# dguilliams3/book-recommendation-engine

Hardware: AMD Instinct MI355X
Metric: exact top-10 queries/sec at 10M×1536 fp32 (1/8 GPU) + % HBM/MFMA roofline (higher is better)
Workload: dtype fp32

## Files before the change

### book-recommendation-engine_amd/csrc/vs_engines.hip

```cpp
#include "vs_host.h"

using namespace vs;
using namespace vs::host;

namespace {

bool env_on(const char* name) {
  const char* e = getenv(name);
  return !e || atoi(e) != 0;
}
int env_int(const char* name, int dflt) {
  const char* e = getenv(name);
  return e ? atoi(e) : dflt;
}

int engine_from_env() {
  const char* e = getenv("VS_ENGINE");
  if (!e) return VS_ENGINE_AUTO;
  if (strcmp(e, "fp32") == 0) return VS_ENGINE_FP32_MFMA;
  if (strcmp(e, "bf16v") == 0) return VS_ENGINE_BF16_VERIFY;
  if (strcmp(e, "i8v") == 0) return VS_ENGINE_I8_VERIFY;
  return VS_ENGINE_AUTO;
}
bool wide_enabled() {
// ... 318 lines not shown
    if (!gathered) x.timing = &tm;
    if (gathered && s.deep && !i8 && s.kmode == MODE_IP && a.self0 < 0 && skinny_deep_on()) {
      VS_HIP(launch_skinny_plane(FILTER_BF16, x.XH, x.QH, x.ld, s.ntotal, s.gc, nullptr, nullptr,
                                 s.part, st),
             "vs: skinny deep stage");
      x.qskip = skinny_plane_max_queries();
    }
    if (s.small) {
      int* cnt = nullptr;
      VS_HIP(s.scr.alloc((void**)&cnt, sizeof(int)), "vs: scratch");
      VS_HIP(hipMemsetD32Async((hipDeviceptr_t)cnt, a.nq, 1, st), "vs: count");
      KernelTimer ks(st, i8 ? "skinny_plane_topk_i8" : "skinny_plane_topk");
      VS_HIP(launch_skinny_plane(s.plane, x.XH, x.QH, x.ld, s.ntotal, cnt, s.qs, x.xs, s.part, st,
                                 a.nq),
             "vs: skinny first stage");
      ks.stop();
    } else {
      int nd = 0;
      VS_HIP(launch_gemm_topk_x1(s.kmode, x, s.part, st, &nd), "vs: gemm_topk_x1 launch");
    }
    x.timing = nullptr;
    whole.stop();
  }
  if (s.aug)
    VS_HIP(launch_l2aug_map(s.part.key, s.part.id, (int64_t)s.part.P * s.part.KP, s.qa_rows,
                            s.qaux, s.idx->aug.nref, x.qcut, st),
           "vs: L2 keys");
  return VS_OK;
}

int merge_and_verify(Stage& s) {
  vs_index* idx = s.idx;
  const SearchArgs& a = s.a;
  Scratch& scr = s.scr;
  hipStream_t st = s.st;
  const Partials& part = s.part;
  const int nq = s.nq, KF = s.KF, L = s.L;
  float* Dk = nullptr;
  int64_t* Ik = nullptr;
  VS_HIP(scr.alloc((void**)&Dk, (size_t)nq * KF * sizeof(float)), "vs: scratch");
  VS_HIP(scr.alloc((void**)&Ik, (size_t)nq * KF * sizeof(int64_t)), "vs: scratch");
  if (KF > 64) {
    VS_HIP(launch_select_lists(part, L, nq, KF, Dk, Ik, st, s.gc), "vs: merge");
  } else if (select_heads_applies(part, L, KF)) {
    VS_HIP(launch_select_heads(part, nq, KF, Dk, Ik, st, s.gc), "vs: merge");
  } else {
    Partials mp = part;
    mp.KP = kp_for(KF);
    mp.KL = L;
    VS_HIP(launch_merge_partials(MODE_L2, mp, nq, KF, 0, 0.0f, Dk, Ik, KF, st, 0, nullptr, s.gc),
           "vs: merge");
  }
  Partials vp;
  vp.KP = kp_for(KF);
  vp.P = 1;
  int* flags = nullptr;
  VS_HIP(scr.alloc((void**)&vp.key, (size_t)nq * vp.KP * sizeof(float)), "vs: scratch");
  VS_HIP(scr.alloc((void**)&vp.id, (size_t)nq * vp.KP * sizeof(int)), "vs: scratch");
  VS_HIP(scr.alloc((void**)&flags, (size_t)nq * sizeof(int)), "vs: scratch");
  VS_HIP(scr.alloc((void**)&s.qlist, (size_t)s.x.nq_pad * sizeof(int)), "vs: scratch");
  VS_HIP(scr.alloc((void**)&s.qcount, 2 * sizeof(int)), "vs: scratch");
  VerifyArgs v;
  v.mode = s.vmode;
  v.KF = KF;
  v.M = s.need;
  v.X = idx->codes;
  v.xesize = idx->esize;
  v.xn = idx->norms;
  v.Q = s.Q;
  v.qn = s.qaux;
  v.ld = idx->ld;
  v.ba = s.ba;
  v.stats = s.stats;
  v.lists = part;
  v.L = L;
  v.okey = vp.key;
  v.oid = vp.id;
  v.KP = vp.KP;
  v.fail = flags;
  v.qinv = a.mode == MODE_COS ? s.qaux : nullptr;
  v.xinv = a.mode == MODE_COS ? a.xaux : nullptr;
  v.qr2i8 = s.qr2;
  v.qcut = s.x.qcut;
  VS_HIP(launch_verify_rescore(v, nq, Dk, Ik, s.gc, st), "vs: verify");
  unsigned long long* dst = device_stats(idx->device);
  if (!dst) return fail(VS_E_HIP, "vs: statistics buffer");
  VS_HIP(launch_compact_flags(flags, nq, s.qlist, s.qcount, dst + 1,
                              s.gathered ? nullptr : dst + 0, st),
         "vs: flags");
  if (wide_enabled())
    VS_HIP(launch_verify_wide(v, nq, s.qlist, s.qcount, Dk, Ik, dst + 4, st), "vs: verify wide");
  VS_HIP(launch_compact_flags(flags, nq, s.qlist, s.qcount + 1,
                              s.last_plane ? dst + 2 : dst + 3, nullptr, st),
         "vs: flags");
  VS_HIP(launch_merge_partials(s.vmode, vp, nq, a.k, idx->id_base, a.min_score, a.D, a.I, a.k, st,
                               a.raw, s.gl, s.gc),
         "vs: merge");
  return VS_OK;
}

int hand_off(Stage& s) {
  vs_index* idx = s.idx;
  const SearchArgs& a = s.a;
  hipStream_t st = s.st;
  const int* left_count = s.qcount + 1;
  int left = -1;
  if ((!s.gathered || s.deep) && tail_wait_on(a, st)) {
    int rc = read_count(left_count, st, &left);
    if (rc) return rc;
  }
  if (!s.last_plane && !s.gathered && s.plane == FILTER_I8) {
    int rc = adaptive_record(idx, left_count, s.nq, st);
    if (rc) return rc;
  }
  if (left == 0) return VS_OK;
  const int* next = s.qlist;
  if (s.gathered) {
    int* composed = nullptr;
    VS_HIP(s.scr.alloc((void**)&composed, (size_t)s.x.nq_pad * sizeof(int)), "vs: scratch");
    VS_HIP(launch_compose_list(s.gl, s.qlist, left_count, s.x.nq_pad, composed, st), "vs: flags");
    next = composed;
  }
  if (!s.last_plane)
    return run_filter_verify(idx, a, s.need, s.KF, st, FILTER_BF16, true, true, next, left_count);
  return run_gemm_rescored(idx, a, s.need, s.KF, s.plane, st, next, left_count);
}

int run_filter_verify(vs_index* idx, const SearchArgs& a, int need, int KF, hipStream_t st,
                      int plane, bool last_plane, bool deep, const int* gl, const int* gc) {
  Stage s(idx, a, need, KF, st, plane, last_plane, deep, gl, gc);
  int rc = size_lists(s);
  if (!rc) rc = stage_queries(s);
  if (!rc) rc = arm_dumps(s);
  if (!rc) rc = run_pass(s);
  if (!rc) rc = merge_and_verify(s);
  if (!rc) rc = hand_off(s);
  return rc;
}

constexpr int kExactSlots = 256;
constexpr int kXPageSlots = 1024;

int run_gemm_rescored(vs_index* idx, const SearchArgs& a, int need, int KF, int plane,
                      hipStream_t st, const int* gl, const int* gc) {
  if (KF > 64) return run_paged(idx, a, st, gl, gc);
  const int ntotal = (int)idx->ntotal;
  const int KP = kp_for(KF);
  const int nslot = (int)round_up(a.nq, kBQ);
  Partials part;
  part.KP = KP;
  const int ntiles = (ntotal + kBN - 1) / kBN;
  const int nsplit = gathered_nsplit(ntiles);
  part.P = 2 * nsplit;
  const int cap = slot_window_cap(nslot, part.P, KP);
  Scratch scr(st);
  const size_t n = (size_t)cap * part.P * KP;
  VS_HIP(scr.alloc((void**)&part.key, n * sizeof(float)), "vs: scratch");
  VS_HIP(scr.alloc((void**)&part.id, n * sizeof(int)), "vs: scratch");
  float *qc = nullptr, *ac = nullptr;
  int* qrow = nullptr;
  VS_HIP(scr.alloc((void**)&qc, (size_t)cap * idx->ld * sizeof(float)), "vs: scratch");
  VS_HIP(scr.alloc((void**)&ac, (size_t)cap * sizeof(float)), "vs: scratch");
  VS_HIP(scr.alloc((void**)&qrow, (size_t)cap * sizeof(int)), "vs: scratch");
  float* Dk = nullptr;
  int64_t* Ik = nullptr;
  VS_HIP(scr.alloc((void**)&Dk, (size_t)cap * KF * sizeof(float)), "vs: scratch");
// ... 424 lines not shown
```

### book-recommendation-engine_amd/csrc/vs_internal.h

```cpp
#pragma once

#include <hip/hip_runtime.h>

#include <cfloat>
#include <climits>
#include <cstdint>

namespace vs {

enum Mode : int { MODE_IP = 0, MODE_L2 = 1, MODE_COS = 2, MODE_L2D = 3 };

constexpr int kBN = 128;
constexpr int kBQ = 128;
constexpr int kBK = 32;
constexpr int kRowPad = 256;
constexpr int kGemvMaxQ = 8;
constexpr int kBlasThreshold = 20;
constexpr int kSkinnyMaxQ = 32;

__host__ __device__ inline uint16_t f32_to_bf16_rne(float f) {
  uint32_t u;
  __builtin_memcpy(&u, &f, 4);
  if ((u & 0x7F800000u) == 0x7F800000u && (u & 0x007FFFFFu))
    return (uint16_t)((u >> 16) | 0x0040u);
// ... 36 lines not shown
  virtual void end(hipStream_t st) = 0;
  virtual ~X1Timing() = default;
};
struct X1Args {
  X1Timing* timing = nullptr;
  int qskip = 0;
  int filter = FILTER_BF16;
  const void* XH = nullptr;
  const float* xs = nullptr;
  const float* xgmax = nullptr;
  const float* xgmin = nullptr;
  bool dump = false;
  bool dump32 = false;
  float* qcut = nullptr;
  const double* qbkey = nullptr;
  int qcut_m = 0;
  int recut = 1;
  const float* ecut_x = nullptr;
  const float* ecut_q = nullptr;
  int64_t ecut_ld = 0;
  float* qam = nullptr;
  float* ecut_key = nullptr;
  int* ecut_id = nullptr;
  int* dcount = nullptr;
  int* dslot = nullptr;
  int dR = 0;
  unsigned long long* dstats = nullptr;
  const float* xaux = nullptr;
  const void* QH = nullptr;
  int qtile0 = 0;
  const float* qs = nullptr;
  const float* qaux = nullptr;
  int nqa = 0;
  int64_t ld = 0;
  int ntotal = 0;
  int nq_pad = 0;
  int nsplit = 1;
  int64_t self0 = -1;
  const int* qrow = nullptr;
  const int* qcount = nullptr;
};
constexpr int kX1Q = 256;
constexpr int kEcutMaxM = 32;
constexpr int64_t kI8MaxLd = 131072;
int x1_list_len(int need);
int x1_lane_len();
hipError_t x1_stamps(unsigned long long* out, int reset);
bool x1_plan_describe(int mode, int filter, int64_t ntotal, int nsplit, bool can_dump, bool ecut,
                      bool gathered, int recut, bool dump32, int32_t* out, int cap, int* nlaunch);
hipError_t launch_gemm_topk_x1(int mode, const X1Args& a, Partials part, hipStream_t st,
                               int* ndispatch);
struct BoundArgs {
  int filter = FILTER_BF16;
  double gam = 0.0;
  double norm_inf = 0.0;
  int l2aug = 0;
  double aug_q2 = 0.0;
  double aug_nref = 0.0;
  int rows_exact = 0;
};
BoundArgs make_bound_args(int64_t ld, int filter);
struct VerifyArgs {
  int mode = MODE_IP;
  int KF = 0;
  int M = 0;
  const void* X = nullptr;
  int xesize = 4;
  const float* xn = nullptr;
  const float* Q = nullptr;
  const float* qn = nullptr;
  int64_t ld = 0;
  BoundArgs ba;
  const unsigned* stats = nullptr;
  Partials lists;
  int L = 0;
  float* okey = nullptr;
  int* oid = nullptr;
  int KP = 0;
  int* fail = nullptr;
  const float* qinv = nullptr;
  const float* xinv = nullptr;
  const float* qr2i8 = nullptr;
  const float* qcut = nullptr;
};
struct L2Aug {
  int m = 0;
  float C = 0.0f;
  float nref = 0.0f;
  float Cb = 0.0f;
};
constexpr int kAugBf16 = 64;
BoundArgs make_bound_args_l2aug(int64_t ld, const L2Aug& g, int filter = FILTER_I8);
hipError_t launch_bound_stats(const float* norms, const float* rn2, int64_t n, unsigned* out,
                              hipStream_t st, bool accumulate = false);
hipError_t launch_resid_norms(const float* X, int64_t ld, int64_t r0, int64_t n, float* out,
                              hipStream_t st);
hipError_t launch_quantize_i8(const void* X, int64_t ld, int64_t r0, int64_t n, int8_t* codes,
                              float* scale, float* rn2, hipStream_t st, int xesize = 4);
hipError_t launch_quantize_i8_l2aug(const float* X, int64_t ld, int64_t r0, int64_t n,
                                    const L2Aug& g, const float* norms, int8_t* codes,
                                    float* scale, float* rn2, float* anorm, hipStream_t st);
hipError_t launch_bf16_plane_l2aug(const float* X, int64_t ld, int64_t r0, int64_t n,
                                   const L2Aug& g, const float* norms, uint16_t* plane, float* rn2,
                                   float* anorm, hipStream_t st);
hipError_t l2aug_params(const float* X, int64_t ld, int64_t r0, int64_t n, const float* norms,
                        L2Aug* out, hipStream_t st);
hipError_t launch_l2aug_map(float* key, const int* id, int64_t per_query, int nq,
                            const float* qn, float nref, float* qcut, hipStream_t st);
hipError_t launch_gather_queries(const float* src, int64_t ld, const float* aux, const int* gl,
                                 const int* count, int nslot, int64_t self0, float* dst,
                                 float* daux, int* drow, hipStream_t st);
hipError_t launch_add_counts(const int* count, int n, unsigned long long* acc, hipStream_t st);
hipError_t launch_compose_list(const int* outer, const int* inner, const int* count, int n,
                               int* out, hipStream_t st);
hipError_t launch_window_count(const int* count, int w0, int cap, int* out, hipStream_t st);
hipError_t launch_group_max(const float* f, int64_t n, float* out, hipStream_t st,
                            int64_t nvalid = 0, float* outmin = nullptr);
hipError_t launch_mul_arrays(const float* a, const float* b, int64_t n, float* out,
                             hipStream_t st);
hipError_t launch_verify_rescore(const VerifyArgs& v, int nq, const float* Dk, const int64_t* Ik,
                                 const int* qcount, hipStream_t st);
hipError_t launch_compact_flags(const int* flags, int n, int* list, int* count,
                                unsigned long long* total, unsigned long long* total_n,
                                hipStream_t st);
constexpr int kWideCap = 4096;
hipError_t launch_verify_wide(const VerifyArgs& v, int nq_max, const int* qlist, const int* count,
                              const float* Dk, const int64_t* Ik, unsigned long long* sizes,
                              hipStream_t st);
constexpr int kVerifyMaxKF = 1024;
hipError_t launch_select_lists(Partials part, int L, int nq, int KF, float* Dk, int64_t* Ik,
                               hipStream_t st, const int* qcount = nullptr);
bool select_heads_applies(const Partials& part, int L, int KF);
hipError_t launch_select_heads(Partials part, int nq, int KF, float* Dk, int64_t* Ik,
                               hipStream_t st, const int* qcount = nullptr);

struct ScratchChunk {
  void* p = nullptr;
  size_t size = 0;
  int dev = 0;
  hipEvent_t ev = nullptr;
  hipStream_t st = nullptr;
};
hipError_t scratch_chunk_get(size_t bytes, hipStream_t st, ScratchChunk* out);
void scratch_chunk_put(const ScratchChunk& c, hipStream_t st);
void scratch_trim();
hipError_t launch_qbound(int mode, const float* Q, int64_t ld, const float* qn, int filter,
                         const unsigned* stats, const float* qr2i8, int nq, double* bkey,
                         hipStream_t st, const BoundArgs* ba = nullptr);
bool x1_dump_applies(int mode, int filter);
int x1_dump_slots();
bool x1_pass_dumps(int ntotal, int nsplit);
hipError_t launch_x1_replay(const X1Args& a, Partials part, hipStream_t st);
hipError_t launch_merge_partials(int mode, Partials part, int nq, int k, int64_t id_base,
                                 float min_score, float* D, int64_t* I, int64_t ldo,
                                 hipStream_t st, int raw = 0, const int* qlist = nullptr,
                                 const int* qcount = nullptr);
hipError_t launch_merge_parts(int mode, const float* Dp, const int64_t* Ip, int nparts,
                              int nq, int k_in, int k, float* D, int64_t* I, hipStream_t st);
struct ExactStreamArgs {
  const float* X = nullptr;
  const float* xn = nullptr;
  const float* xinv = nullptr;
  int64_t ld = 0;
  int ntotal = 0;
  const float* Q = nullptr;
  const float* qaux = nullptr;
// ... 300 lines not shown
```

### book-recommendation-engine_amd/csrc/vs_x1_device.h

```cpp
#pragma once

#include "vs_device.h"

namespace vs {

__device__ __forceinline__ f32x4 row4(const float* __restrict__ p) { return *(const f32x4*)p; }
__device__ __forceinline__ f32x4 row4(const uint16_t* __restrict__ p) {
  const uint2 u = *(const uint2*)p;
  return f32x4{__uint_as_float(u.x << 16), __uint_as_float(u.x & 0xFFFF0000u),
               __uint_as_float(u.y << 16), __uint_as_float(u.y & 0xFFFF0000u)};
}

template <int EL>
__device__ __forceinline__ float x1_key(int sum_bits, float qsc, float fx) {
  if constexpr (EL == FILTER_I8) return -((float)sum_bits * (qsc * fx));
  else return -__int_as_float(sum_bits);
}

__device__ __forceinline__ uint32_t key_order(float f) {
  const uint32_t u = __float_as_uint(f);
  return (u & 0x80000000u) ? ~u : (u | 0x80000000u);
}
__device__ __forceinline__ float key_unorder(uint32_t u) {
  return __uint_as_float((u & 0x80000000u) ? (u & 0x7FFFFFFFu) : ~u);
}

template <bool DIFF = false, typename RT = float>
__device__ __forceinline__ double wave_dot(const RT* __restrict__ x, const float* __restrict__ q,
                                           int64_t ld, int lane) {
  double acc = 0.0;
  for (int64_t c = lane * 4; c < ld; c += 256) {
    const f32x4 xv = row4(x + c);
    const f32x4 qv = *(const f32x4*)(q + c);
#pragma unroll
    for (int e = 0; e < 4; ++e) {
      if constexpr (DIFF) {
        const double t = (double)xv[e] - (double)qv[e];
        acc = fma(t, t, acc);
      } else {
        acc = fma((double)xv[e], (double)qv[e], acc);
      }
    }
  }
  for (int o = 32; o > 0; o >>= 1) acc += __shfl_xor(acc, o);
  return acc;
}

constexpr int kQV = 8;
struct QSlice {
  f32x4 v[kQV];
};
__device__ __forceinline__ void load_qslice(const float* __restrict__ q, int64_t ld, int lane,
                                            QSlice& qs) {
#pragma unroll
  for (int i = 0; i < kQV; ++i) {
    const int64_t c = lane * 4 + 256 * i;
    qs.v[i] = c < ld ? *(const f32x4*)(q + c) : f32x4{0.f, 0.f, 0.f, 0.f};
  }
}
template <bool DIFF = false, typename RT = float>
__device__ __forceinline__ void wave_dot2(const RT* __restrict__ xa, const RT* __restrict__ xb,
                                          const QSlice& qs, int64_t ld, int lane, double& ra,
                                          double& rb) {
  f32x4 va[kQV], vb[kQV];
#pragma unroll
  for (int i = 0; i < kQV; ++i) {
    const int64_t c = lane * 4 + 256 * i;
    va[i] = c < ld ? row4(xa + c) : f32x4{0.f, 0.f, 0.f, 0.f};
    vb[i] = c < ld ? row4(xb + c) : f32x4{0.f, 0.f, 0.f, 0.f};
  }
  double a = 0.0, b = 0.0;
#pragma unroll
  for (int i = 0; i < kQV; ++i) {
    if (lane * 4 + 256 * i >= ld) break;
#pragma unroll
    for (int e = 0; e < 4; ++e) {
      if constexpr (DIFF) {
        const double ta = (double)va[i][e] - (double)qs.v[i][e];
        const double tb = (double)vb[i][e] - (double)qs.v[i][e];
        a = fma(ta, ta, a);
        b = fma(tb, tb, b);
      } else {
        a = fma((double)va[i][e], (double)qs.v[i][e], a);
        b = fma((double)vb[i][e], (double)qs.v[i][e], b);
      }
    }
  }
  for (int o = 32; o > 0; o >>= 1) {
    a += __shfl_xor(a, o);
    b += __shfl_xor(b, o);
  }
  ra = a;
  rb = b;
}

template <int MODE>
__device__ __forceinline__ float exact_key(float ip, int q, int r, const float* __restrict__ qn,
                                           const float* __restrict__ xn,
                                           const float* __restrict__ qinv,
                                           const float* __restrict__ xinv) {
  return MODE == MODE_L2    ? l2_from_ip(qn[q], xn[r], ip)
         : MODE == MODE_COS ? -(ip * (qinv[q] * xinv[r]))
         : MODE == MODE_L2D ? ip
                            : -ip;
}


__device__ __forceinline__ void replay_stats(int cnt, int dR,
                                             unsigned long long* __restrict__ stats) {
  unsigned long long a = (unsigned long long)cnt, b = cnt > dR ? 1ull : 0ull;
  for (int o = 32; o > 0; o >>= 1) {
    a += __shfl_xor(a, o);
    b += __shfl_xor(b, o);
  }
  if ((threadIdx.x & 63) == 0 && a && stats) {
    atomicAdd(stats, a);
    if (b) atomicAdd(stats + 1, b);
  }
}

template <int KR>
__device__ __forceinline__ void lane_list_load(const float* __restrict__ pkey,
                                               const int* __restrict__ pid, int64_t o,
                                               float (&lk)[KR], int (&li)[KR]) {
  static_assert(KR % 4 == 0, "lane lists move as 16-B pieces");
#pragma unroll
  for (int e = 0; e < KR; e += 4) {
    const f32x4 kv = *(const f32x4*)(pkey + o + e);
    const int4 iv = *(const int4*)(pid + o + e);
    lk[e] = kv.x, lk[e + 1] = kv.y, lk[e + 2] = kv.z, lk[e + 3] = kv.w;
    li[e] = iv.x, li[e + 1] = iv.y, li[e + 2] = iv.z, li[e + 3] = iv.w;
  }
}
template <int KR>
__device__ __forceinline__ void lane_list_store(float* __restrict__ pkey, int* __restrict__ pid,
                                                int64_t o, const float (&lk)[KR],
                                                const int (&li)[KR]) {
#pragma unroll
  for (int e = 0; e < KR; e += 4) {
    *(f32x4*)(pkey + o + e) = f32x4{lk[e], lk[e + 1], lk[e + 2], lk[e + 3]};
    *(int4*)(pid + o + e) = make_int4(li[e], li[e + 1], li[e + 2], li[e + 3]);
  }
}

template <int KR, int EL>
__device__ __forceinline__ void replay_admit(float (&lk)[KR], int (&li)[KR],
                                             const int* __restrict__ dslot, int64_t i, int64_t nl,
                                             int cnt, float qsc, const float* __restrict__ xs,
                                             int selfrow, int ntotal, float cut) {
  const i32x2* sl = (const i32x2*)dslot + i;
  constexpr int kB = 8;
  for (int c0 = 0; c0 < cnt; c0 += kB) {
    i32x2 e[kB];
    float fx[kB];
#pragma unroll
    for (int j = 0; j < kB; ++j) e[j] = c0 + j < cnt ? sl[(int64_t)(c0 + j) * nl] : i32x2{-1, 0};
#pragma unroll
    for (int j = 0; j < kB; ++j)
      fx[j] = EL == FILTER_I8 && e[j][0] >= 0 && e[j][0] < ntotal ? xs[e[j][0]] : 0.0f;
#pragma unroll
    for (int j = 0; j < kB; ++j) {
      const int row = e[j][0];
      if (!(row >= 0 && row < ntotal && row != selfrow)) continue;
      const float key = x1_key<EL>(e[j][1], qsc, fx[j]);
      if (key < fminf(lk[KR - 1], cut)) list_insert<KR, int>(lk, li, key, row);
    }
  }
}

__device__ __forceinline__ float lower_cut(float base, double factor, double B, float old) {
  const double tp = (double)base + factor * B;
  if (isfinite(tp) && tp < (double)FLT_MAX) {
    float t = (float)tp;
    if ((double)t < tp) t = nextafterf(t, INFINITY);
    if (t < old) return t;
  }
  return old;
}
// ... 7 lines not shown
```

### book-recommendation-engine_amd/csrc/vs_x1_verify.hip

```cpp
#include <algorithm>
#include <climits>
#include <cmath>
#include <cstdlib>

#include "vs_x1_device.h"

namespace vs {



__device__ __forceinline__ double bound_key(int mode, const BoundArgs& ba, double qh2, double qr2,
                                            double qn2, const unsigned* stats) {
  if (ba.l2aug) {
    const double ax2 = (double)__uint_as_float(stats[0]);
    const double hx = sqrt(ax2) + sqrt((double)__uint_as_float(stats[1]));
    const double rx = sqrt((double)__uint_as_float(stats[1]));
    const double hq = sqrt(qh2), rq = sqrt(qr2);
    const double u = ldexp(1.0, -24);
    double b = ba.gam * hx * hq + hx * rq + rx * hq + rx * rq;
    b *= 1.0 + 1e-6;
    double B = 2.0 * b + 8.0 * u * (qn2 + ax2) + 2.0 * u * (qn2 + ba.aug_nref + 2.01 * hx * hq);
    if (mode == MODE_L2D) B += (ba.norm_inf + 4.0 * u) * (qn2 + ax2);
    return B * (1.0 + 1e-6);
  }
  const double xm = sqrt((double)__uint_as_float(stats[0]) * (1.0 + ba.norm_inf));
  const double rx = ba.rows_exact ? 0.0 : sqrt((double)__uint_as_float(stats[1]));
  const double hx = xm + rx;
  const double hq = sqrt(qh2), rq = sqrt(qr2), qn = sqrt(qn2);
  double b = ba.gam * hx * hq + hx * rq + rx * hq + rx * rq + 2.0 * ldexp(1.0, -24) * xm * qn;
  b *= 1.0 + 1e-6;
  if (mode == MODE_L2 || mode == MODE_L2D) {
    const double xm2 = (double)__uint_as_float(stats[0]);
    b = 2.0 * b + 8.0 * ldexp(1.0, -24) * (qn2 + xm2);
    if (mode == MODE_L2D) b += (ba.norm_inf + 4.0 * ldexp(1.0, -24)) * (qn2 + xm2);
  } else if (mode == MODE_COS) {
    const double rho =
        ba.rows_exact ? 0.0 : sqrt((double)__uint_as_float(stats[2]) * (1.0 + ba.norm_inf));
    const double rel = ba.gam * (1 + rho) * (1 + rho) + 2 * rho * (1 + rho) + rho * rho +
                       ldexp(1.0, -23);
    b = (rel * (1.0 + 1.5 * ba.norm_inf) + ldexp(1.0, -22)) * (1.0 + 1e-6);
  }
  return b;
}

__device__ __forceinline__ void query_split_norms(const float* __restrict__ qrow, int64_t ld,
                                                  int lane, const float* __restrict__ qr2i8,
                                                  double& qh2, double& qr2, double& qn2,
                                                  double aug = 0.0) {
  double a = 0.0, r = 0.0, n = 0.0;
  for (int64_t c = lane * 4; c < ld; c += 256) {
    const f32x4 v = *(const f32x4*)(qrow + c);
#pragma unroll
    for (int i = 0; i < 4; ++i) {
      const float x = v[i];
      const float hi = __uint_as_float((uint32_t)f32_to_bf16_rne(x) << 16);
      const double rr = (double)x - (double)hi;
      a += (double)hi * hi;
      r += rr * rr;
      n += (double)x * x;
    }
  }
  for (int o = 32; o > 0; o >>= 1) {
    a += __shfl_xor(a, o);
    r += __shfl_xor(r, o);
    n += __shfl_xor(n, o);
  }
  qh2 = a + aug;
  qr2 = r;
  qn2 = n;
  if (qr2i8) {
    qr2 = (double)*qr2i8;
    const double hq = sqrt(n + aug) + sqrt(qr2);
    qh2 = hq * hq;
  }
}

template <int MODE, int NE, typename RT>
__global__ __launch_bounds__(64) void verify_rescore_kernel(
    int KF, int M, const float* __restrict__ Dk, const int64_t* __restrict__ Ik,
    const RT* __restrict__ X, const float* __restrict__ xn, const float* __restrict__ Q,
    const float* __restrict__ qn, int64_t ld, BoundArgs ba, const unsigned* __restrict__ stats,
    const float* __restrict__ lkey, const int* __restrict__ lid, int P, int LKP, int L,
    float* __restrict__ okey, int* __restrict__ oid, int KP, int* __restrict__ fail,
    const float* __restrict__ qinv, const float* __restrict__ xinv, const float* __restrict__ qr2i8,
    const int* __restrict__ qcount, const float* __restrict__ qcut) {
  __shared__ float ek[64 * NE];
  __shared__ int sid[64 * NE];
  __shared__ float eMs;
  const int lane = threadIdx.x;
  const int q = blockIdx.x;
  if (qcount && q >= *qcount) {
    if (lane == 0) fail[q] = 0;
    return;
  }
  int id[NE];
#pragma unroll
  for (int e = 0; e < NE; ++e) {
    const int j = lane + 64 * e;
    id[e] = j < KF ? (int)Ik[(int64_t)q * KF + j] : -1;
    sid[j] = id[e];
  }
  if (lane == 0) eMs = FLT_MAX;
  const float aK = Dk[(int64_t)q * KF + KF - 1];
  const int idK = (int)Ik[(int64_t)q * KF + KF - 1];
  bool bounded = idK >= 0;
  float T = idK >= 0 ? aK : FLT_MAX;
  for (int j = lane; j < P; j += 64) {
    const int64_t o = ((int64_t)q * P + j) * LKP + L - 1;
    if (lid[o] >= 0) {
      bounded = true;
      T = fminf(T, lkey[o]);
    }
  }
  for (int o = 32; o > 0; o >>= 1) T = fminf(T, __shfl_xor(T, o));
  bounded = __any(bounded);
  if (qcut && qcut[q] < FLT_MAX) {
    bounded = true;
    T = fminf(T, qcut[q]);
  }

  const float* qrow = Q + (int64_t)q * ld;
  double qh2, qr2, qn2;
  query_split_norms(qrow, ld, lane, qr2i8 ? qr2i8 + q : nullptr, qh2, qr2, qn2, ba.aug_q2);
  if (ba.rows_exact) {
    qh2 = qn2;
    qr2 = 0.0;
  }
  __syncthreads();
  if (ld <= 256 * kQV) {
    QSlice qsl;
    load_qslice(qrow, ld, lane, qsl);
    for (int j = 0; j < KF; j += 2) {
      const int ra = sid[j], rb = j + 1 < KF ? sid[j + 1] : -1;
      double da, db;
      wave_dot2<MODE == MODE_L2D, RT>(X + (int64_t)max(ra, 0) * ld, X + (int64_t)max(rb, 0) * ld,
                                      qsl, ld, lane, da, db);
      if (lane == 0) {
        ek[j] = ra < 0 ? FLT_MAX : exact_key<MODE>((float)da, q, ra, qn, xn, qinv, xinv);
        if (j + 1 < KF) ek[j + 1] = rb < 0 ? FLT_MAX : exact_key<MODE>((float)db, q, rb, qn, xn, qinv, xinv);
      }
    }
  } else {
    for (int j = 0; j < KF; ++j) {
      const int r = sid[j];
      if (r < 0) {
        if (lane == 0) ek[j] = FLT_MAX;
        continue;
      }
      const double acc = wave_dot<MODE == MODE_L2D, RT>(X + (int64_t)r * ld, qrow, ld, lane);
      if (lane == 0) ek[j] = exact_key<MODE>((float)acc, q, r, qn, xn, qinv, xinv);
    }
  }
  __syncthreads();
  float* ok = okey + (int64_t)q * KP;
  int* oi = oid + (int64_t)q * KP;
#pragma unroll
  for (int e = 0; e < NE; ++e) {
    const int s = lane + 64 * e;
    if (s < KF) {
      const float k0 = ek[s];
      const int i0 = id[e] < 0 ? INT_MAX : id[e];
      int rank = 0;
      for (int j = 0; j < KF; ++j) {
        const float kj = ek[j];
        const int ij = sid[j] < 0 ? INT_MAX : sid[j];
        rank += (lex_less(kj, ij, k0, i0) || (kj == k0 && ij == i0 && j < s)) ? 1 : 0;
      }
      ok[rank] = k0;
      oi[rank] = id[e];
      if (rank == M - 1) eMs = k0;
    } else if (s < KP) {
      ok[s] = FLT_MAX;
      oi[s] = -1;
    }
  }
  __syncthreads();
  const float eM = eMs;
  const double bkey = bound_key(MODE, ba, qh2, qr2,
                                MODE == MODE_L2 || MODE == MODE_L2D ? (double)qn[q] : qn2, stats);
  const bool pass = !bounded || ((double)T - bkey > (double)eM && isfinite(T) && isfinite(eM) &&
                                  isfinite(bkey));
  if (lane == 0) fail[q] = pass ? 0 : 1;
}

hipError_t launch_verify_rescore(const VerifyArgs& v, int nq, const float* Dk, const int64_t* Ik,
                                 const int* qcount, hipStream_t st) {
  const int KF = v.KF;
  if (KF > kVerifyMaxKF || v.KP > kVerifyMaxKF || KF > v.KP || v.M < 1 || v.M > KF ||
      v.ld % 4 != 0 || v.L < 1 || v.L > v.lists.KP || (v.xesize != 4 && v.xesize != 2))
    return hipErrorInvalidValue;
  if (nq <= 0) return hipSuccess;
#define VS_VERIFY_T(MD, NE, RT)                                                                   \
  hipLaunchKernelGGL((verify_rescore_kernel<MD, NE, RT>), dim3(nq), dim3(64), 0, st, KF, v.M, Dk, \
                     Ik, (const RT*)v.X, v.xn, v.Q, v.qn, v.ld, v.ba, v.stats, v.lists.key,       \
                     v.lists.id, v.lists.P, v.lists.KP, v.L, v.okey, v.oid, v.KP, v.fail, v.qinv, \
                     v.xinv, v.qr2i8, qcount, v.qcut)
#define VS_VERIFY(MD, NE)                  \
  do {                                     \
    if (v.xesize == 4)                     \
      VS_VERIFY_T(MD, NE, float);          \
    else                                   \
      VS_VERIFY_T(MD, NE, uint16_t);       \
  } while (0)
#define VS_VERIFY_NE(MD)   \
  do {                     \
    if (KF <= 64)          \
      VS_VERIFY(MD, 1);    \
    else if (KF <= 128)    \
      VS_VERIFY(MD, 2);    \
    else if (KF <= 256)    \
      VS_VERIFY(MD, 4);    \
    else if (KF <= 512)    \
      VS_VERIFY(MD, 8);    \
    else                   \
      VS_VERIFY(MD, 16);   \
  } while (0)
  if (v.mode == MODE_IP)
    VS_VERIFY_NE(MODE_IP);
  else if (v.mode == MODE_L2)
    VS_VERIFY_NE(MODE_L2);
  else if (v.mode == MODE_L2D)
    VS_VERIFY_NE(MODE_L2D);
  else if (v.mode == MODE_COS && v.qinv && v.xinv)
    VS_VERIFY_NE(MODE_COS);
  else
    return hipErrorInvalidValue;
#undef VS_VERIFY_NE
#undef VS_VERIFY
#undef VS_VERIFY_T
  return hipGetLastError();
}

__global__ __launch_bounds__(1024) void compact_flags_kernel(const int* __restrict__ flags, int n,
                                                             int* __restrict__ list,
                                                             int* __restrict__ count,
                                                             unsigned long long* __restrict__ total,
                                                             unsigned long long* __restrict__ total_n) {
  __shared__ int wsum[16];
  __shared__ int base;
  const int tid = threadIdx.x, lane = tid & 63, wv = tid >> 6;
  if (tid == 0) base = 0;
  __syncthreads();
  for (int c0 = 0; c0 < n; c0 += 1024) {
    const int i = c0 + tid;
    const int f = i < n && flags[i] != 0 ? 1 : 0;
    const uint64_t bal = __ballot(f);
    const int before = __popcll(bal & ((1ull << lane) - 1ull));
    if (lane == 0) wsum[wv] = __popcll(bal);
    __syncthreads();
    int off = base;
    for (int j = 0; j < wv; ++j) off += wsum[j];
    if (f) list[off + before] = i;
    __syncthreads();
    if (tid == 0) {
      int s = 0;
      for (int j = 0; j < 16; ++j) s += wsum[j];
      base += s;
    }
    __syncthreads();
  }
  if (tid == 0) {
    *count = base;
    if (total) atomicAdd(total, (unsigned long long)base);
    if (total_n) atomicAdd(total_n, (unsigned long long)n);
  }
}

__global__ void add_counts_kernel(const int* __restrict__ count, int n,
                                  unsigned long long* __restrict__ acc) {
  atomicAdd(acc + 0, (unsigned long long)n);
  atomicAdd(acc + 1, (unsigned long long)*count);
}

hipError_t launch_add_counts(const int* count, int n, unsigned long long* acc, hipStream_t st) {
  hipLaunchKernelGGL(add_counts_kernel, dim3(1), dim3(1), 0, st, count, n, acc);
  return hipGetLastError();
}

hipError_t launch_compact_flags(const int* flags, int n, int* list, int* count,
                                unsigned long long* total, unsigned long long* total_n,
                                hipStream_t st) {
  if (n < 0) return hipErrorInvalidValue;
  hipLaunchKernelGGL(compact_flags_kernel, dim3(1), dim3(1024), 0, st, flags, n, list, count,
                     total, total_n);
  return hipGetLastError();
}

template <int MODE, typename RT>
__global__ __launch_bounds__(256) void verify_wide_kernel(
    const int* __restrict__ qlist, const int* __restrict__ count, int KF, int M,
    const RT* __restrict__ X, const float* __restrict__ xn, const float* __restrict__ Q,
    const float* __restrict__ qn, int64_t ld, BoundArgs ba, const unsigned* __restrict__ stats,
    const float* __restrict__ lkey, const int* __restrict__ lid, int P, int LKP, int L,
    float* __restrict__ okey, int* __restrict__ oid, int KP, int* __restrict__ fail,
    const float* __restrict__ qinv, const float* __restrict__ xinv, const float* __restrict__ qr2i8,
    const float* __restrict__ Dk, const int64_t* __restrict__ Ik,
    unsigned long long* __restrict__ sizes, const float* __restrict__ qcut) {
  __shared__ float ck[kWideCap];
  __shared__ int cid[kWideCap];
  __shared__ float rk[kVerifyMaxKF], kk[kVerifyMaxKF];
  __shared__ int ri[kVerifyMaxKF], ki[kVerifyMaxKF];
  __shared__ int cntk;
  __shared__ float wT[4];
  __shared__ int wB[4];
  __shared__ int cnt, bad;
  __shared__ float eMs;
  __shared__ double qs[3];
  const int tid = threadIdx.x, lane = tid & 63, wv = tid >> 6;
  const int nflag = *count;
  for (int jq = blockIdx.x; jq < nflag; jq += gridDim.x) {
    const int q = qlist[jq];
    const int64_t lbase = (int64_t)q * P * LKP;
    float T = FLT_MAX;
    bool bounded = false;
    for (int j = tid; j < P; j += 256) {
      const int64_t o = lbase + (int64_t)j * LKP + L - 1;
      if (lid[o] >= 0) {
        bounded = true;
        T = fminf(T, lkey[o]);
      }
    }
    for (int o = 32; o > 0; o >>= 1) T = fminf(T, __shfl_xor(T, o));
    bounded = __any(bounded);
    if (lane == 0) {
      wT[wv] = T;
      wB[wv] = bounded ? 1 : 0;
    }
    if (tid == 0) {
      cnt = 0;
      cntk = 0;
      bad = 0;
      eMs = FLT_MAX;
    }
    for (int t = tid; t < kVerifyMaxKF; t += 256) {
      rk[t] = t < KP ? okey[(int64_t)q * KP + t] : FLT_MAX;
      ri[t] = t < KP ? oid[(int64_t)q * KP + t] : -1;
    }
    const float* qrow = Q + (int64_t)q * ld;
    if (wv == 0) {
      double a, b, c;
      query_split_norms(qrow, ld, lane, qr2i8 ? qr2i8 + q : nullptr, a, b, c, ba.aug_q2);
      if (lane == 0) {
        qs[0] = a;
        qs[1] = b;
        qs[2] = c;
      }
    }
    __syncthreads();
    T = fminf(fminf(wT[0], wT[1]), fminf(wT[2], wT[3]));
    bounded = (wB[0] | wB[1] | wB[2] | wB[3]) != 0;
    if (qcut && qcut[q] < FLT_MAX) {
      bounded = true;
      T = fminf(T, qcut[q]);
    }
    const double bkey =
        bound_key(MODE, ba, qs[0], qs[1],
                  MODE == MODE_L2 || MODE == MODE_L2D ? (double)qn[q] : qs[2], stats);
    if (bounded && Dk) {
      const float aM = Dk[(int64_t)q * KF + M - 1];
      double tp = (double)aM + 2.000001 * bkey;
      if (ri[M - 1] >= 0 && isfinite(rk[M - 1]))
        tp = fmin(tp, (double)rk[M - 1] + 1.000001 * bkey);
      if (isfinite(tp) && tp < (double)T) {
        float t = (float)tp;
        if ((double)t < tp) t = nextafterf(t, INFINITY);
        T = fminf(T, t);
      }
    }
    const float kfk = Dk ? Dk[(int64_t)q * KF + KF - 1] : -FLT_MAX;
    const int kfi = Dk ? (int)Ik[(int64_t)q * KF + KF - 1] : INT_MIN;
    for (int j = tid; j < P * L; j += 256) {
      const int64_t o = lbase + (int64_t)(j / L) * LKP + j % L;
      const int r = lid[o];
      const float lk = lkey[o];
      if (r >= 0 && (!bounded || lk < T)) {
        int hit = -1;
        if (Dk && (kfi < 0 || !lex_less(kfk, kfi, lk, r)))
          for (int t = 0; t < KP; ++t) hit = ri[t] == r ? t : hit;
        if (hit >= 0) {
          const int s = atomicAdd(&cntk, 1);
          if (s < kVerifyMaxKF) {
            kk[s] = rk[hit];
            ki[s] = r;
          }
        } else {
          const int s = atomicAdd(&cnt, 1);
          if (s < kWideCap) cid[s] = r;
        }
      }
    }
    __syncthreads();
    const int nu = cnt;
    const int nk = min(cntk, kVerifyMaxKF);
    const int n = nu + cntk;
    if (sizes && tid == 0) {
      atomicAdd(sizes, (unsigned long long)n);
      atomicAdd(sizes + 1, (unsigned long long)nu);
    }
    if (!(n > kWideCap || n < M || !isfinite(T))) {
      auto put = [&](int j, int r, double acc) {
        if (lane == 0) {
          const float key = exact_key<MODE>((float)acc, q, r, qn, xn, qinv, xinv);
          ck[j] = key;
          if (!isfinite(key)) bad = 1;
        }
      };
      if (ld <= 256 * kQV) {
        QSlice qsl;
        load_qslice(qrow, ld, lane, qsl);
        for (int j = wv; j < nu; j += 8) {
          const int ra = cid[j], rb = j + 4 < nu ? cid[j + 4] : ra;
          double da, db;
          wave_dot2<MODE == MODE_L2D, RT>(X + (int64_t)ra * ld, X + (int64_t)rb * ld, qsl, ld, lane, da,
                                      db);
          put(j, ra, da);
          if (j + 4 < nu) put(j + 4, rb, db);
        }
      } else {
        for (int j = wv; j < nu; j += 4) {
          const int r = cid[j];
          put(j, r, wave_dot<MODE == MODE_L2D, RT>(X + (int64_t)r * ld, qrow, ld, lane));
        }
      }
      for (int t = tid; t < nk; t += 256) {
        ck[nu + t] = kk[t];
        cid[nu + t] = ki[t];
        if (!isfinite(kk[t])) bad = 1;
      }
      __syncthreads();
      if (!bad) {
        float* ok = okey + (int64_t)q * KP;
        int* oi = oid + (int64_t)q * KP;
        for (int j = tid; j < n; j += 256) {
          const float kj = ck[j];
          const int ij = cid[j];
          int rank = 0;
          for (int t = 0; t < n; ++t) rank += lex_less(ck[t], cid[t], kj, ij) ? 1 : 0;
          if (rank < KF) {
            ok[rank] = kj;
            oi[rank] = ij;
          }
          if (rank == M - 1) eMs = kj;
        }
        for (int j = min(n, KF) + tid; j < KP; j += 256) {
          ok[j] = FLT_MAX;
          oi[j] = -1;
        }
        __syncthreads();
        const float eM = eMs;
        const bool pass =
            !bounded || ((double)T - bkey > (double)eM && isfinite(eM) && isfinite(bkey));
        if (tid == 0 && pass) fail[q] = 0;
      }
    }
    __syncthreads();
  }
}

hipError_t launch_verify_wide(const VerifyArgs& v, int nq_max, const int* qlist, const int* count,
                              const float* Dk, const int64_t* Ik, unsigned long long* sizes,
                              hipStream_t st) {
  if (v.KF > v.KP || v.KP > kVerifyMaxKF || (Dk && !Ik) || v.M < 1 || v.M > v.KF ||
      v.ld % 4 != 0 || v.L < 1 || v.L > v.lists.KP || (v.xesize != 4 && v.xesize != 2))
    return hipErrorInvalidValue;
  if (nq_max <= 0) return hipSuccess;
  const int grid = std::min(nq_max, 2048);
#define VS_WIDE_T(MD, RT)                                                                        \
  hipLaunchKernelGGL((verify_wide_kernel<MD, RT>), dim3(grid), dim3(256), 0, st, qlist, count,   \
                     v.KF, v.M, (const RT*)v.X, v.xn, v.Q, v.qn, v.ld, v.ba, v.stats,            \
                     v.lists.key, v.lists.id, v.lists.P, v.lists.KP, v.L, v.okey, v.oid, v.KP,   \
                     v.fail, v.qinv, v.xinv, v.qr2i8, Dk, Ik, sizes, v.qcut)
#define VS_WIDE(MD)             \
  do {                          \
    if (v.xesize == 4)          \
      VS_WIDE_T(MD, float);     \
    else                        \
      VS_WIDE_T(MD, uint16_t);  \
  } while (0)
  if (v.mode == MODE_IP)
    VS_WIDE(MODE_IP);
  else if (v.mode == MODE_L2)
    VS_WIDE(MODE_L2);
  else if (v.mode == MODE_L2D)
    VS_WIDE(MODE_L2D);
  else if (v.mode == MODE_COS && v.qinv && v.xinv)
    VS_WIDE(MODE_COS);
  else
    return hipErrorInvalidValue;
#undef VS_WIDE
#undef VS_WIDE_T
  return hipGetLastError();
}

template <int MODE>
__global__ __launch_bounds__(64) void qbound_kernel(const float* __restrict__ Q, int64_t ld,
                                                    const float* __restrict__ qn, BoundArgs ba,
                                                    const unsigned* __restrict__ stats,
                                                    const float* __restrict__ qr2i8, int nq,
                                                    double* __restrict__ bkey) {
  const int q = blockIdx.x;
  const int lane = threadIdx.x;
  if (q >= nq) return;
  double qh2, qr2, qn2;
  query_split_norms(Q + (int64_t)q * ld, ld, lane, qr2i8 ? qr2i8 + q : nullptr, qh2, qr2, qn2,
                    ba.aug_q2);
  if (ba.rows_exact) {
    qh2 = qn2;
    qr2 = 0.0;
  }
  double b = bound_key(MODE, ba, qh2, qr2,
                                MODE == MODE_L2 || MODE == MODE_L2D ? (double)qn[q] : qn2, stats);
  if (ba.l2aug) b *= 0.5;
  if (lane == 0) bkey[q] = b;
}

hipError_t launch_qbound(int mode, const float* Q, int64_t ld, const float* qn, int filter,
                         const unsigned* stats, const float* qr2i8, int nq, double* bkey,
                         hipStream_t st, const BoundArgs* bap) {
  if (nq <= 0) return hipSuccess;
  if (ld % 4 != 0) return hipErrorInvalidValue;
  const BoundArgs ba = bap ? *bap : make_bound_args(ld, filter);
#define VS_QB(MD) \
  hipLaunchKernelGGL(qbound_kernel<MD>, dim3(nq), dim3(64), 0, st, Q, ld, qn, ba, stats, qr2i8, nq, bkey)
  if (mode == MODE_IP)
    VS_QB(MODE_IP);
  else if (mode == MODE_L2)
    VS_QB(MODE_L2);
  else if (mode == MODE_COS)
    VS_QB(MODE_COS);
  else if (mode == MODE_L2D)
    VS_QB(MODE_L2D);
  else
    return hipErrorInvalidValue;
#undef VS_QB
  return hipGetLastError();
}

__global__ __launch_bounds__(256) void select_lists_kernel(const float* __restrict__ lkey,
                                                           const int* __restrict__ lid, int P,
                                                           int LKP, int L, int KF,
                                                           float* __restrict__ Dk,
                                                           int64_t* __restrict__ Ik,
                                                           const int* __restrict__ qcount) {
  __shared__ int wsum[4];
  __shared__ unsigned long long sel[kVerifyMaxKF];
  __shared__ int nsel;
  __shared__ int hist[256];
  __shared__ int sel_digit, sel_before;
  const int q = blockIdx.x;
  const int tid = threadIdx.x, lane = tid & 63, wv = tid >> 6;
  if (qcount && q >= *qcount) return;
  const int64_t base = (int64_t)q * P * LKP;
  const int n = P * L;
  constexpr int kR = 16;
  constexpr unsigned long long kNone = ~0ull;
  unsigned long long v[kR];
  const bool regs = n <= 256 * kR;
  auto image = [&](int j) -> unsigned long long {
    const int64_t o = base + (int64_t)(j / L) * LKP + j % L;
    const int r = lid[o];
    return r >= 0 ? ((unsigned long long)key_order(lkey[o]) << 32) | (uint32_t)r : kNone;
  };
#pragma unroll
  for (int i = 0; i < kR; ++i) {
    const int j = tid + 256 * i;
    v[i] = regs && j < n ? image(j) : kNone;
  }
  auto count_le = [&](unsigned long long y) {
    int c = 0;
    if (regs) {
#pragma unroll
      for (int i = 0; i < kR; ++i) c += v[i] <= y && v[i] != kNone ? 1 : 0;
    } else {
// ... 221 lines not shown
```

Measured before the change: 86700.

## Rescore four rows per wave, stage query in LDS, reuse exact keys from ecut

New measurement: 87020, median of 6. About the same (+0.4%).

```diff
diff --git a/book-recommendation-engine_amd/csrc/vs_engines.hip b/book-recommendation-engine_amd/csrc/vs_engines.hip
--- a/book-recommendation-engine_amd/csrc/vs_engines.hip
+++ b/book-recommendation-engine_amd/csrc/vs_engines.hip
@@ -424,6 +424,11 @@
   v.xinv = a.mode == MODE_COS ? a.xaux : nullptr;
   v.qr2i8 = s.qr2;
   v.qcut = s.x.qcut;
+  if (s.x.ecut_key && s.x.ecut_id && s.vmode == MODE_IP && idx->esize == 4 &&
+      s.x.ecut_x == (const float*)idx->codes && s.x.ecut_q == s.Q) {
+    v.ekey = s.x.ecut_key;
+    v.eid = s.x.ecut_id;
+  }
   VS_HIP(launch_verify_rescore(v, nq, Dk, Ik, s.gc, st), "vs: verify");
   unsigned long long* dst = device_stats(idx->device);
   if (!dst) return fail(VS_E_HIP, "vs: statistics buffer");
diff --git a/book-recommendation-engine_amd/csrc/vs_internal.h b/book-recommendation-engine_amd/csrc/vs_internal.h
--- a/book-recommendation-engine_amd/csrc/vs_internal.h
+++ b/book-recommendation-engine_amd/csrc/vs_internal.h
@@ -142,6 +142,8 @@
   const float* xinv = nullptr;
   const float* qr2i8 = nullptr;
   const float* qcut = nullptr;
+  const float* ekey = nullptr;
+  const int* eid = nullptr;
 };
 struct L2Aug {
   int m = 0;
diff --git a/book-recommendation-engine_amd/csrc/vs_x1_device.h b/book-recommendation-engine_amd/csrc/vs_x1_device.h
--- a/book-recommendation-engine_amd/csrc/vs_x1_device.h
+++ b/book-recommendation-engine_amd/csrc/vs_x1_device.h
@@ -94,6 +94,47 @@
   rb = b;
 }
 
+template <bool DIFF, typename RT, int NV>
+__device__ __forceinline__ void wave_dot4(const RT* __restrict__ x0, const RT* __restrict__ x1,
+                                          const RT* __restrict__ x2, const RT* __restrict__ x3,
+                                          const float* qv, int64_t ld, int lane, double (&r)[4]) {
+  static_assert(NV <= kQV, "the rows' register slices");
+  const RT* const x[4] = {x0, x1, x2, x3};
+  f32x4 v[4][NV];
+#pragma unroll
+  for (int i = 0; i < NV; ++i) {
+    const int64_t c = lane * 4 + 256 * i;
+#pragma unroll
+    for (int k = 0; k < 4; ++k) v[k][i] = c < ld ? row4(x[k] + c) : f32x4{0.f, 0.f, 0.f, 0.f};
+  }
+  double acc[4] = {0.0, 0.0, 0.0, 0.0};
+#pragma unroll
+  for (int i = 0; i < NV; ++i) {
+    const int64_t c = lane * 4 + 256 * i;
+    if (c >= ld) break;
+    const f32x4 qq = *(const f32x4*)(qv + c);
+#pragma unroll
+    for (int e = 0; e < 4; ++e) {
+#pragma unroll
+      for (int k = 0; k < 4; ++k) {
+        if constexpr (DIFF) {
+          const double t = (double)v[k][i][e] - (double)qq[e];
+          acc[k] = fma(t, t, acc[k]);
+        } else {
+          acc[k] = fma((double)v[k][i][e], (double)qq[e], acc[k]);
+        }
+      }
+    }
+  }
+  for (int o = 32; o > 0; o >>= 1) {
+#pragma unroll
+    for (int k = 0; k < 4; ++k) acc[k] += __shfl_xor(acc[k], o);
+  }
+#pragma unroll
+  for (int k = 0; k < 4; ++k) r[k] = acc[k];
+}
+__host__ __device__ constexpr int dot4_nv(int64_t ld) { return ld <= 256 * 6 ? 6 : kQV; }
+
 template <int MODE>
 __device__ __forceinline__ float exact_key(float ip, int q, int r, const float* __restrict__ qn,
                                            const float* __restrict__ xn,
diff --git a/book-recommendation-engine_amd/csrc/vs_x1_verify.hip b/book-recommendation-engine_amd/csrc/vs_x1_verify.hip
--- a/book-recommendation-engine_amd/csrc/vs_x1_verify.hip
+++ b/book-recommendation-engine_amd/csrc/vs_x1_verify.hip
@@ -75,7 +75,7 @@
   }
 }
 
-template <int MODE, int NE, typename RT>
+template <int MODE, int NE, typename RT, int NV>
 __global__ __launch_bounds__(64) void verify_rescore_kernel(
     int KF, int M, const float* __restrict__ Dk, const int64_t* __restrict__ Ik,
     const RT* __restrict__ X, const float* __restrict__ xn, const float* __restrict__ Q,
@@ -83,9 +83,14 @@
     const float* __restrict__ lkey, const int* __restrict__ lid, int P, int LKP, int L,
     float* __restrict__ okey, int* __restrict__ oid, int KP, int* __restrict__ fail,
     const float* __restrict__ qinv, const float* __restrict__ xinv, const float* __restrict__ qr2i8,
-    const int* __restrict__ qcount, const float* __restrict__ qcut) {
+    const int* __restrict__ qcount, const float* __restrict__ qcut,
+    const float* __restrict__ ekey, const int* __restrict__ eid) {
   __shared__ float ek[64 * NE];
   __shared__ int sid[64 * NE];
+  __shared__ int todo[64 * NE];
+  __shared__ __attribute__((aligned(16))) float qv[256 * NV];
+  __shared__ float kkey[kEcutMaxM];
+  __shared__ int kid[kEcutMaxM];
   __shared__ float eMs;
   const int lane = threadIdx.x;
   const int q = blockIdx.x;
@@ -93,12 +98,18 @@
     if (lane == 0) fail[q] = 0;
     return;
   }
+  constexpr bool kKept = MODE == MODE_IP && sizeof(RT) == 4;
+  const bool kept = kKept && ekey && eid;
   int id[NE];
 #pragma unroll
   for (int e = 0; e < NE; ++e) {
     const int j = lane + 64 * e;
     id[e] = j < KF ? (int)Ik[(int64_t)q * KF + j] : -1;
     sid[j] = id[e];
+  }
+  if (kept && lane < kEcutMaxM) {
+    kid[lane] = eid[(int64_t)q * kEcutMaxM + lane];
+    kkey[lane] = ekey[(int64_t)q * kEcutMaxM + lane];
   }
   if (lane == 0) eMs = FLT_MAX;
   const float aK = Dk[(int64_t)q * KF + KF - 1];
@@ -120,6 +131,9 @@
   }
 
   const float* qrow = Q + (int64_t)q * ld;
+  const bool quads = ld <= 256 * NV;
+  if (quads)
+    for (int64_t c = lane * 4; c < ld; c += 256) *(f32x4*)(qv + c) = *(const f32x4*)(qrow + c);
   double qh2, qr2, qn2;
   query_split_norms(qrow, ld, lane, qr2i8 ? qr2i8 + q : nullptr, qh2, qr2, qn2, ba.aug_q2);
   if (ba.rows_exact) {
@@ -127,26 +141,47 @@
     qr2 = 0.0;
   }
   __syncthreads();
-  if (ld <= 256 * kQV) {
-    QSlice qsl;
-    load_qslice(qrow, ld, lane, qsl);
-    for (int j = 0; j < KF; j += 2) {
-      const int ra = sid[j], rb = j + 1 < KF ? sid[j + 1] : -1;
-      double da, db;
-      wave_dot2<MODE == MODE_L2D, RT>(X + (int64_t)max(ra, 0) * ld, X + (int64_t)max(rb, 0) * ld,
-                                      qsl, ld, lane, da, db);
+  int nt = 0;
+#pragma unroll
+  for (int e = 0; e < NE; ++e) {
+    const int j = lane + 64 * e;
+    bool need = false;
+    if (j < KF) {
+      float key = FLT_MAX;
+      need = id[e] >= 0;
+      if (kept && need) {
+        for (int t = 0; t < kEcutMaxM; ++t)
+          if (kid[t] == id[e]) key = kkey[t], need = false;
+      }
+      if (!need) ek[j] = key;
+    }
+    const uint64_t bal = __ballot(need);
+    if (need) todo[nt + __popcll(bal & ((1ull << lane) - 1ull))] = j;
+    nt += __popcll(bal);
+  }
+  __syncthreads();
+  if (quads) {
+    for (int t = 0; t < nt; t += 4) {
+      int js[4], rs[4];
+#pragma unroll
+      for (int k = 0; k < 4; ++k) {
+        js[k] = todo[min(t + k, nt - 1)];
+        rs[k] = __builtin_amdgcn_readfirstlane(sid[js[k]]);
+      }
+      double d[4];
+      wave_dot4<MODE == MODE_L2D, RT, NV>(X + (int64_t)rs[0] * ld, X + (int64_t)rs[1] * ld,
+                                           X + (int64_t)rs[2] * ld, X + (int64_t)rs[3] * ld, qv, ld,
+                                           lane, d);
       if (lane == 0) {
-        ek[j] = ra < 0 ? FLT_MAX : exact_key<MODE>((float)da, q, ra, qn, xn, qinv, xinv);
-        if (j + 1 < KF) ek[j + 1] = rb < 0 ? FLT_MAX : exact_key<MODE>((float)db, q, rb, qn, xn, qinv, xinv);
+#pragma unroll
+        for (int k = 0; k < 4; ++k)
+          if (t + k < nt) ek[js[k]] = exact_key<MODE>((float)d[k], q, rs[k], qn, xn, qinv, xinv);
       }
     }
   } else {
-    for (int j = 0; j < KF; ++j) {
+    for (int t = 0; t < nt; ++t) {
+      const int j = todo[t];
       const int r = sid[j];
-      if (r < 0) {
-        if (lane == 0) ek[j] = FLT_MAX;
-        continue;
-      }
       const double acc = wave_dot<MODE == MODE_L2D, RT>(X + (int64_t)r * ld, qrow, ld, lane);
       if (lane == 0) ek[j] = exact_key<MODE>((float)acc, q, r, qn, xn, qinv, xinv);
     }
@@ -190,11 +225,18 @@
       v.ld % 4 != 0 || v.L < 1 || v.L > v.lists.KP || (v.xesize != 4 && v.xesize != 2))
     return hipErrorInvalidValue;
   if (nq <= 0) return hipSuccess;
-#define VS_VERIFY_T(MD, NE, RT)                                                                   \
-  hipLaunchKernelGGL((verify_rescore_kernel<MD, NE, RT>), dim3(nq), dim3(64), 0, st, KF, v.M, Dk, \
-                     Ik, (const RT*)v.X, v.xn, v.Q, v.qn, v.ld, v.ba, v.stats, v.lists.key,       \
+#define VS_VERIFY_NV(MD, NE, RT, NV)                                                              \
+  hipLaunchKernelGGL((verify_rescore_kernel<MD, NE, RT, NV>), dim3(nq), dim3(64), 0, st, KF, v.M, \
+                     Dk, Ik, (const RT*)v.X, v.xn, v.Q, v.qn, v.ld, v.ba, v.stats, v.lists.key,   \
                      v.lists.id, v.lists.P, v.lists.KP, v.L, v.okey, v.oid, v.KP, v.fail, v.qinv, \
-                     v.xinv, v.qr2i8, qcount, v.qcut)
+                     v.xinv, v.qr2i8, qcount, v.qcut, v.ekey, v.eid)
+#define VS_VERIFY_T(MD, NE, RT)          \
+  do {                                   \
+    if (dot4_nv(v.ld) == 6)              \
+      VS_VERIFY_NV(MD, NE, RT, 6);       \
+    else                                 \
+      VS_VERIFY_NV(MD, NE, RT, kQV);     \
+  } while (0)
 #define VS_VERIFY(MD, NE)                  \
   do {                                     \
     if (v.xesize == 4)                     \
@@ -228,6 +270,7 @@
 #undef VS_VERIFY_NE
 #undef VS_VERIFY
 #undef VS_VERIFY_T
+#undef VS_VERIFY_NV
   return hipGetLastError();
 }
 
@@ -286,8 +329,8 @@
   return hipGetLastError();
 }
 
-template <int MODE, typename RT>
-__global__ __launch_bounds__(256) void verify_wide_kernel(
+template <int MODE, typename RT, int NV>
+__global__ __launch_bounds__(256, NV <= 6 ? 3 : 2) void verify_wide_kernel(
     const int* __restrict__ qlist, const int* __restrict__ count, int KF, int M,
     const RT* __restrict__ X, const float* __restrict__ xn, const float* __restrict__ Q,
     const float* __restrict__ qn, int64_t ld, BoundArgs ba, const unsigned* __restrict__ stats,
@@ -298,17 +341,23 @@
     unsigned long long* __restrict__ sizes, const float* __restrict__ qcut) {
   __shared__ float ck[kWideCap];
   __shared__ int cid[kWideCap];
-  __shared__ float rk[kVerifyMaxKF], kk[kVerifyMaxKF];
-  __shared__ int ri[kVerifyMaxKF], ki[kVerifyMaxKF];
+  extern __shared__ __attribute__((aligned(16))) float wide_lds[];
+  float* rk = wide_lds;
+  float* kk = rk + KP;
+  int* ri = (int*)(kk + KP);
+  int* ki = ri + KP;
+  float* qv = (float*)(ki + KP);
   __shared__ int cntk;
   __shared__ float wT[4];
   __shared__ int wB[4];
   __shared__ int cnt, bad;
   __shared__ float eMs;
   __shared__ double qs[3];
-  const int tid = threadIdx.x, lane = tid & 63, wv = tid >> 6;
   const int nflag = *count;
   for (int jq = blockIdx.x; jq < nflag; jq += gridDim.x) {
+    int tid = threadIdx.x;
+    asm volatile("" : "+v"(tid));
+    const int lane = tid & 63, wv = __builtin_amdgcn_readfirstlane(tid >> 6);
     const int q = qlist[jq];
     const int64_t lbase = (int64_t)q * P * LKP;
     float T = FLT_MAX;
@@ -332,11 +381,14 @@
       bad = 0;
       eMs = FLT_MAX;
     }
-    for (int t = tid; t < kVerifyMaxKF; t += 256) {
-      rk[t] = t < KP ? okey[(int64_t)q * KP + t] : FLT_MAX;
-      ri[t] = t < KP ? oid[(int64_t)q * KP + t] : -1;
+    for (int t = tid; t < KP; t += 256) {
+      rk[t] = okey[(int64_t)q * KP + t];
+      ri[t] = oid[(int64_t)q * KP + t];
     }
     const float* qrow = Q + (int64_t)q * ld;
+    const bool quads = ld <= 256 * NV;
+    if (quads)
+      for (int64_t c = tid * 4; c < ld; c += 1024) *(f32x4*)(qv + c) = *(const f32x4*)(qrow + c);
     if (wv == 0) {
       double a, b, c;
       query_split_norms(qrow, ld, lane, qr2i8 ? qr2i8 + q : nullptr, a, b, c, ba.aug_q2);
@@ -379,7 +431,7 @@
           for (int t = 0; t < KP; ++t) hit = ri[t] == r ? t : hit;
         if (hit >= 0) {
           const int s = atomicAdd(&cntk, 1);
-          if (s < kVerifyMaxKF) {
+          if (s < KP) {
             kk[s] = rk[hit];
             ki[s] = r;
           }
@@ -391,7 +443,7 @@
     }
     __syncthreads();
     const int nu = cnt;
-    const int nk = min(cntk, kVerifyMaxKF);
+    const int nk = min(cntk, KP);
     const int n = nu + cntk;
     if (sizes && tid == 0) {
       atomicAdd(sizes, (unsigned long long)n);
@@ -405,16 +457,19 @@
           if (!isfinite(key)) bad = 1;
         }
       };
-      if (ld <= 256 * kQV) {
-        QSlice qsl;
-        load_qslice(qrow, ld, lane, qsl);
-        for (int j = wv; j < nu; j += 8) {
-          const int ra = cid[j], rb = j + 4 < nu ? cid[j + 4] : ra;
-          double da, db;
-          wave_dot2<MODE == MODE_L2D, RT>(X + (int64_t)ra * ld, X + (int64_t)rb * ld, qsl, ld, lane, da,
-                                      db);
-          put(j, ra, da);
-          if (j + 4 < nu) put(j + 4, rb, db);
+      if (quads) {
+        for (int j = wv; j < nu; j += 16) {
+          int rs[4];
+#pragma unroll
+          for (int k = 0; k < 4; ++k)
+            rs[k] = __builtin_amdgcn_readfirstlane(cid[j + 4 * k < nu ? j + 4 * k : j]);
+          double d[4];
+          wave_dot4<MODE == MODE_L2D, RT, NV>(X + (int64_t)rs[0] * ld, X + (int64_t)rs[1] * ld,
+                                               X + (int64_t)rs[2] * ld, X + (int64_t)rs[3] * ld, qv,
+                                               ld, lane, d);
+#pragma unroll
+          for (int k = 0; k < 4; ++k)
+            if (j + 4 * k < nu) put(j + 4 * k, rs[k], d[k]);
         }
       } else {
         for (int j = wv; j < nu; j += 4) {
@@ -465,11 +520,20 @@
     return hipErrorInvalidValue;
   if (nq_max <= 0) return hipSuccess;
   const int grid = std::min(nq_max, 2048);
-#define VS_WIDE_T(MD, RT)                                                                        \
-  hipLaunchKernelGGL((verify_wide_kernel<MD, RT>), dim3(grid), dim3(256), 0, st, qlist, count,   \
-                     v.KF, v.M, (const RT*)v.X, v.xn, v.Q, v.qn, v.ld, v.ba, v.stats,            \
+  const int nv = dot4_nv(v.ld);
+  const size_t lds = 16 * (size_t)v.KP + (v.ld <= 256 * nv ? 4 * (size_t)v.ld : 0);
+#define VS_WIDE_NV(MD, RT, NV)                                                                   \
+  hipLaunchKernelGGL((verify_wide_kernel<MD, RT, NV>), dim3(grid), dim3(256), lds, st, qlist,    \
+                     count, v.KF, v.M, (const RT*)v.X, v.xn, v.Q, v.qn, v.ld, v.ba, v.stats,     \
                      v.lists.key, v.lists.id, v.lists.P, v.lists.KP, v.L, v.okey, v.oid, v.KP,   \
                      v.fail, v.qinv, v.xinv, v.qr2i8, Dk, Ik, sizes, v.qcut)
+#define VS_WIDE_T(MD, RT)        \
+  do {                           \
+    if (nv == 6)                 \
+      VS_WIDE_NV(MD, RT, 6);     \
+    else                         \
+      VS_WIDE_NV(MD, RT, kQV);   \
+  } while (0)
 #define VS_WIDE(MD)             \
   do {                          \
     if (v.xesize == 4)          \
@@ -489,6 +553,7 @@
     return hipErrorInvalidValue;
 #undef VS_WIDE
 #undef VS_WIDE_T
+#undef VS_WIDE_NV
   return hipGetLastError();
 }
 
```
